# gisbi-kim/navtech-radar-slam

Measured on AMD Instinct MI355X. Metric: sc_loop_queries_per_sec_vs_10k_scan_db, higher is better.
Workload: dtype f16 filter + f64 exact

## Files before the change

### navtech-radar-slam_amd/csrc/sc_window.hip

```cpp
#include <hip/hip_runtime.h>

#include <cmath>
#include <cstdint>

#include "rsx_common.h"
#include "sc_kernels.h"
#include "sc_entry_dev.h"
#include "sc_window_dev.h"

namespace rsx {
namespace sc {

namespace {

using win::half8;
using win::floatx16;
using win::u64;
using win::kNonFinite;
using win::W_STEPS;
using win::W_TILE1;
using win::QK_COPY;
using win::QK_LO;
using win::QK_NORM;
using win::W_LDS;

constexpr int W_ST2_OFF = DS * 2, W_QM_OFF = W_ST2_OFF + 2 * 128 * 2;
static_assert(W_ST2_OFF % 16 == 0 && W_QM_OFF % 8 == 0 && W_QM_OFF + 8 <= 5 * WINDOW_P * 4, "staging fits the arrays it aliases");

#ifndef WIN_OCC
#define WIN_OCC 4
#endif
#ifndef WIN_RING
#define WIN_RING 15
#endif
__global__ __launch_bounds__(256) void sc_win_db_keys_kernel(const double *__restrict__ vkey, int64_t first, int64_t count,
                                                             _Float16 *__restrict__ vk16, float *__restrict__ vk_n) {
  const int lane = threadIdx.x & 63, wave = threadIdx.x >> 6;
  const int64_t it = (int64_t)blockIdx.x * 4 + wave;
  if (it >= count) return;
  dev::win_db_keys_entry(vkey, first + it, vk16, vk_n, lane);
}

struct WindowArgs {
  const char *hnR;
  const char *vk16;
  const float *vk_n;
  const u64 *cmask;
  const float *qdesc;
  const double *qnorm;
  const double *qvkey;
  const RescoreEntry *slist;
  const int32_t *sl_cnt;
  WindowPreview *out;
  WindowSurvivor *surv;
  double eps;
  int32_t k;
};

__global__ __launch_bounds__(256, WIN_OCC) void sc_window_kernel(WindowArgs a) {
  extern __shared__ __attribute__((aligned(16))) char smem[];
  __shared__ float s_ub[WINDOW_HEAD];
  __shared__ int s_pos[WINDOW_P];
  __shared__ int s_n2;
  __shared__ float s_tau;
  __shared__ __attribute__((aligned(16))) char s_rec[5 * WINDOW_P * 4];
  float *const s_lb = reinterpret_cast<float *>(s_rec), *const s_pv = s_lb + WINDOW_P, *const s_cand = s_pv + WINDOW_P;
  int *const s_slot = reinterpret_cast<int *>(s_cand + WINDOW_P), *const s_ks = s_slot + WINDOW_P;
  const int lane = threadIdx.x & 63, wave = __builtin_amdgcn_readfirstlane(threadIdx.x >> 6);
  const int qi = blockIdx.x;
  const int sl_cnt = a.sl_cnt[qi];
  WindowSurvivor *list = a.surv + (int64_t)qi * WINDOW_LIST_STRIDE;
  if (sl_cnt <= 0) {
    if (threadIdx.x == 0) {
      WindowListHeader h;
      h.count = 0;
      h.tau_ub = INFINITY;
      h.n_cand = 0;
      h.n_prev = 0;
      *reinterpret_cast<WindowListHeader *>(list) = h;
    }
    return;
  }
  {
    _Float16 *st = reinterpret_cast<_Float16 *>(s_rec);
    _Float16(*st2)[128] = reinterpret_cast<_Float16(*)[128]>(s_rec + W_ST2_OFF);
    u64 *s_qm = reinterpret_cast<u64 *>(s_rec + W_QM_OFF);
    dev::KeySplit ksplit{};
    if (wave == 0) {
      bool nonzero = false, bad = false;
      if (lane < NS) dev::normalise_column(a.qdesc + (int64_t)qi * DS + lane * NR, a.qnorm[(int64_t)qi * NS + lane], &st[lane * NR], nonzero, bad);
      u64 m = __ballot(nonzero && lane < NS);
      if (__ballot(bad && lane < NS)) m |= kNonFinite;
      if (lane == 0) *s_qm = m;
    } else if (wave == 1) {
      ksplit = win::query_keys_stage(lane < NS ? a.qvkey[(int64_t)qi * NS + lane] : 0.0, st2, lane);
    }
    __syncthreads();
    dev::img_query_image(st, *s_qm, reinterpret_cast<uint4 *>(smem), threadIdx.x, 256);
    win::query_keys_copies(st2, smem + FILTER_QIMG_BYTES, threadIdx.x, 256);
    if (wave == 1) win::query_keys_norms(ksplit, smem + FILTER_QIMG_BYTES, lane);
  }
  __syncthreads();
  const int n = lane & 31, hh = lane >> 5;
  const RescoreEntry *sl = a.slist + (int64_t)qi * RESCORE_SHORTLIST_CAP;
  const u64 qm = *reinterpret_cast<const u64 *>(smem + FILTER_QIMG_MASK_OFF);
  const float nq_key = *reinterpret_cast<const float *>(smem + FILTER_QIMG_BYTES + QK_NORM);
  const float uq_key = *reinterpret_cast<const float *>(smem + FILTER_QIMG_BYTES + QK_NORM + 4);
  const char *ap = smem + ((n & 1) ? (FILTER_QIMG_ODD + 40 * n - 8) : (40 * n)) + 16 * hh;
  const char *kp = smem + FILTER_QIMG_BYTES + (n & 7) * QK_COPY + ((n & ~7) + 8 * hh) * 2;

  auto lane_again = [&]() -> int {
    int t = threadIdx.x;
    asm volatile("" : "+v"(t));
    return t & 31;
  };
  auto do_group = [&](auto pos_of, bool have, int pos_any) -> float {
    const int64_t slot = sl[have ? pos_of() : pos_any].slot;

    floatx16 k0 = {0}, k1 = {0};
    {
      const char *bk = a.vk16 + slot * 256 + 16 * hh;
      half8 bh[4], bl[4];
#pragma unroll
      for (int s = 0; s < 4; s++) {
        bh[s] = *reinterpret_cast<const half8 *>(bk + 32 * s);
        bl[s] = *reinterpret_cast<const half8 *>(bk + 128 + 32 * s);
      }
#pragma unroll
      for (int s = 0; s < 4; s++) {
        const half8 ah0 = *reinterpret_cast<const half8 *>(kp + 32 * s);
        const half8 al0 = *reinterpret_cast<const half8 *>(kp + QK_LO + 32 * s);
        const half8 ah1 = *reinterpret_cast<const half8 *>(kp + 64 + 32 * s);
        const half8 al1 = *reinterpret_cast<const half8 *>(kp + QK_LO + 64 + 32 * s);
        k0 = __builtin_amdgcn_mfma_f32_32x32x16_f16(ah0, bh[s], k0, 0, 0, 0);
        k1 = __builtin_amdgcn_mfma_f32_32x32x16_f16(ah1, bh[s], k1, 0, 0, 0);
        k0 = __builtin_amdgcn_mfma_f32_32x32x16_f16(ah0, bl[s], k0, 0, 0, 0);
        k1 = __builtin_amdgcn_mfma_f32_32x32x16_f16(ah1, bl[s], k1, 0, 0, 0);
        k0 = __builtin_amdgcn_mfma_f32_32x32x16_f16(al0, bh[s], k0, 0, 0, 0);
        k1 = __builtin_amdgcn_mfma_f32_32x32x16_f16(al1, bh[s], k1, 0, 0, 0);
      }
    }
    u64 win;
    int kstar;
    win::alignment_of(k0, k1, nq_key, uq_key, reinterpret_cast<const float2 *>(a.vk_n)[slot], hh, win, kstar);

    __builtin_amdgcn_sched_barrier(0);
    floatx16 acc0 = {0}, acc1 = {0};
    {
      const char *brow = a.hnR + slot * (2 * DS) + 16 * hh;
      constexpr int R = WIN_RING;
      static_assert(W_STEPS % R == 0, "whole ring turns");
      half8 ring[R];
#pragma unroll
      for (int u = 0; u < R; u++) ring[u] = *reinterpret_cast<const half8 *>(brow + 32 * u);
#pragma unroll 1
      for (int s0 = 0; s0 < W_STEPS - R; s0 += R) {
#pragma unroll
        for (int u = 0; u < R; u++) {
          const half8 a0 = *reinterpret_cast<const half8 *>(ap + 32 * (s0 + u));
          const half8 a1 = *reinterpret_cast<const half8 *>(ap + 32 * (s0 + u + W_TILE1));
          acc0 = __builtin_amdgcn_mfma_f32_32x32x16_f16(a0, ring[u], acc0, 0, 0, 0);
          acc1 = __builtin_amdgcn_mfma_f32_32x32x16_f16(a1, ring[u], acc1, 0, 0, 0);
          ring[u] = *reinterpret_cast<const half8 *>(brow + 32 * (s0 + R + u));
        }
      }
#pragma unroll
      for (int u = 0; u < R; u++) {
        const half8 a0 = *reinterpret_cast<const half8 *>(ap + 32 * (W_STEPS - R + u));
        const half8 a1 = *reinterpret_cast<const half8 *>(ap + 32 * (W_STEPS - R + u + W_TILE1));
        acc0 = __builtin_amdgcn_mfma_f32_32x32x16_f16(a0, ring[u], acc0, 0, 0, 0);
        acc1 = __builtin_amdgcn_mfma_f32_32x32x16_f16(a1, ring[u], acc1, 0, 0, 0);
      }
    }

    __builtin_amdgcn_sched_barrier(0);
    const u64 em = a.cmask[slot];
    u64 qmg = qm;
    asm volatile("" : "+v"(qmg));
    const float pv = win::preview_of(acc0, acc1, qmg, em, win, kstar, hh);
    if (have && hh == 0) {
      const int pos = pos_of();
      WindowPreview o;
      o.pv = pv;
      o.ks = kstar;
      a.out[(int64_t)qi * WINDOW_P + pos] = o;
      s_slot[pos] = (int)slot;
      s_pv[pos] = pv;
      s_ks[pos] = kstar;
    }
    return (have && kstar >= 0 && pv < 3.0e38f) ? pv + WINDOW_MARGIN : INFINITY;
  };

  auto write_list = [&](float tau_head, int n2) {
    const int lim = sl_cnt < WINDOW_P ? sl_cnt : WINDOW_P;
    const int nh = lim < WINDOW_HEAD ? lim : WINDOW_HEAD;
    const unsigned long long below = (1ull << lane) - 1ull;
    auto records = [&](auto f) {
      for (int p0 = 0; p0 < nh; p0 += 64) f(p0 + lane, p0 + lane < nh);
      for (int c0 = 0; c0 < n2; c0 += 64) f(c0 + lane < n2 ? s_pos[c0 + lane] : 0, c0 + lane < n2);
    };
    int nc = 0;
    records([&](int pos, bool in) {
      const float pv = s_pv[pos];
      const float ub = pv + WINDOW_MARGIN;
      const bool c = in && s_ks[pos] >= 0 && pv < 3.0e38f && ub <= tau_head;
      const unsigned long long bal = __ballot(c);
      if (c) s_cand[nc + __popcll(bal & below)] = ub;
      nc += __popcll(bal);
    });
    dev::wave_lds_fence();
    float tau_w = INFINITY;
    if (nc >= a.k) {
      for (int c0 = 0; c0 < nc; c0 += 64) {
        const int i = c0 + lane;
        const float v = i < nc ? s_cand[i] : INFINITY;
        int r = 0;
        for (int j = 0; j < nc; j++) {
          const float x = s_cand[j];
          r += (x < v || (x == v && j < i)) ? 1 : 0;
        }
        const unsigned long long b = __ballot(i < nc && r == a.k - 1);
        if (b) {
          tau_w = __shfl(v, __ffsll((long long)b) - 1);
          break;
        }
      }
    }
    int ns = 0, n_cand = 0, n_prev = 0;
    records([&](int pos, bool in) {
      const float pv = s_pv[pos];
      const int ks = s_ks[pos];
      const bool none = in && !(pv == pv);
      const bool lb_ok = !((double)s_lb[pos] - a.eps > (double)tau_w);
      const bool cand = in && (none || (pv < INFINITY && lb_ok));
      const float lo = none ? -INFINITY : pv - WINDOW_MARGIN;
      const bool sv = cand && !(lo > tau_w);
      const unsigned long long bal = __ballot(sv);
      if (sv) {
        WindowSurvivor e;
        e.lo = lo;
        e.slot = s_slot[pos];
        e.ks = (none || ks < 0) ? -1 : ks;
        e.pos = pos;
        list[1 + ns + __popcll(bal & below)] = e;
      }
      ns += __popcll(bal);
      n_cand += __popcll(__ballot(cand));
      n_prev += __popcll(__ballot(cand && !none));
    });
    if (lane == 0) {
      WindowListHeader h;
      h.count = ns;
      h.tau_ub = tau_w;
      h.n_cand = n_cand;
      h.n_prev = n_prev;
      *reinterpret_cast<WindowListHeader *>(list) = h;
    }
  };

  float tau_ub;
  {
    const int cnt1 = sl_cnt < WINDOW_HEAD ? sl_cnt : WINDOW_HEAD;
    float ub = INFINITY;
    if (wave * 32 < cnt1) ub = do_group([&] { return wave * 32 + lane_again(); }, wave * 32 + n < cnt1, wave * 32);
    if (hh == 0) s_ub[wave * 32 + n] = ub;
    __syncthreads();
    float lbh0 = INFINITY, lbh1 = INFINITY;
    if (wave == 0) {
      if (lane < cnt1) lbh0 = sl[lane].lb;
      if (lane + 64 < cnt1) lbh1 = sl[lane + 64].lb;
    }
    if (sl_cnt <= WINDOW_HEAD) {
      if (wave == 0) {
        s_lb[lane] = lbh0;
        s_lb[lane + 64] = lbh1;
        dev::wave_lds_fence();
        write_list(INFINITY, 0);
      }
      return;
    }

    {
      const float v0 = s_ub[lane], v1 = s_ub[lane + 64];
      int r0 = 0, r1 = 0;
      const float4 *u4 = reinterpret_cast<const float4 *>(s_ub);
#pragma unroll 4
      for (int j = 0; j < WINDOW_HEAD / 4; j++) {
        const float4 u = u4[j];
        const float x[4] = {u.x, u.y, u.z, u.w};
#pragma unroll
        for (int e = 0; e < 4; e++) {
          const int idx = 4 * j + e;
          r0 += (x[e] < v0 || (x[e] == v0 && idx < lane)) ? 1 : 0;
          r1 += (x[e] < v1 || (x[e] == v1 && idx < lane + 64)) ? 1 : 0;
        }
      }
      const int want = a.k - 1;
      const unsigned long long b0 = __ballot(r0 == want), b1 = __ballot(r1 == want);
      const float c0 = __shfl(v0, b0 ? __ffsll((long long)b0) - 1 : 0), c1 = __shfl(v1, b1 ? __ffsll((long long)b1) - 1 : 0);
      tau_ub = b0 ? c0 : c1;
    }
    if (wave == 0) {
      s_lb[lane] = lbh0;
      s_lb[lane + 64] = lbh1;
    }
  }
  if (wave == 0) {
    int n2 = 0;
    const int lim = sl_cnt < WINDOW_P ? sl_cnt : WINDOW_P;
    for (int p0 = WINDOW_HEAD; p0 < lim; p0 += 64) {
      const int pos = p0 + lane;
      bool pass = false;
      if (pos < lim) {
        const float lb = sl[pos].lb;
        s_lb[pos] = lb;
        pass = !((double)lb - a.eps > (double)tau_ub);
        if (!pass) {
          WindowPreview o;
          o.pv = __builtin_nanf("");
          o.ks = -2;
          a.out[(int64_t)qi * WINDOW_P + pos] = o;
        }
      }
      const unsigned long long bal = __ballot(pass);
      if (pass) s_pos[n2 + __popcll(bal & ((1ull << lane) - 1ull))] = pos;
      n2 += __popcll(bal);
    }
    if (lane == 0) {
      s_n2 = n2;
      s_tau = tau_ub;
    }
  }
  __syncthreads();
  const int n2 = s_n2;
  for (int g = wave; g * 32 < n2; g += 4) {
    const bool have = g * 32 + n < n2;
    (void)do_group([&] { return s_pos[g * 32 + lane_again()]; }, have, s_pos[g * 32]);
  }
  __syncthreads();
  if (wave == 0) write_list(s_tau, n2);
}

}

int launch_window_db_keys(const double *vkey, int64_t first, int64_t count, void *vk16, float *vk_n, hipStream_t s) {
  if (count <= 0) return RSX_OK;
  hipLaunchKernelGGL(sc_win_db_keys_kernel, dim3((unsigned)((count + 3) / 4)), dim3(256), 0, s, vkey, first, count,
                     static_cast<_Float16 *>(vk16), vk_n);
  RSX_HIP(hipGetLastError());
  return RSX_OK;
}

int launch_window(const DbView &db, const QueryView &q, const RescoreEntry *slist, const int32_t *sl_cnt,
                  int32_t k, double eps, WindowPreview *out, WindowSurvivor *surv, hipStream_t s) {
  if (q.nq <= 0) return RSX_OK;
  WindowArgs a;
  a.hnR = static_cast<const char *>(db.hnR);
  a.vk16 = static_cast<const char *>(db.vk16);
  a.vk_n = db.vk_n;
  a.cmask = reinterpret_cast<const u64 *>(db.cmask);
  a.qdesc = q.desc;
  a.qnorm = q.norm;
  a.qvkey = q.vkey;
  a.slist = slist;
  a.sl_cnt = sl_cnt;
  a.out = out;
  a.surv = surv;
  a.eps = eps;
  a.k = k < 1 ? 1 : (k > WINDOW_HEAD ? WINDOW_HEAD : k);
  hipLaunchKernelGGL(sc_window_kernel, dim3((unsigned)q.nq), dim3(256), W_LDS, s, a);
  RSX_HIP(hipGetLastError());
  return RSX_OK;
}

const char *window_kernel_name() { return "sc_window_kernel"; }

}
}
```

### navtech-radar-slam_amd/csrc/sc_window_dev.h

```cpp
#pragma once
#include <hip/hip_runtime.h>

#include <cmath>
#include <cstdint>

#include "sc_kernels.h"
#include "sc_entry_dev.h"

namespace rsx {
namespace sc {
namespace win {

typedef _Float16 half8 __attribute__((ext_vector_type(8)));
typedef float floatx16 __attribute__((ext_vector_type(16)));
typedef unsigned long long u64;

constexpr float kWinAlignEps = 3e-5f;
constexpr u64 kNonFinite = 1ull << 63;
constexpr int W_STEPS = DS / 16;
constexpr int W_TILE1 = 40;
constexpr int QK_COPY = 288;
constexpr int QK_LO = 8 * QK_COPY;
constexpr int QK_NORM = 2 * QK_LO;
static_assert(QK_NORM + 16 == WINDOW_QK_BYTES, "layout");
constexpr int W_LDS = FILTER_QIMG_BYTES + WINDOW_QK_BYTES;

template <bool DPP = false>
__device__ __forceinline__ dev::KeySplit query_keys_stage(double v, _Float16 (*st)[128], int lane) {
  const dev::KeySplit k = dev::split_key<DPP>(lane < NS ? v : 0.0, lane);
  if (lane < NS) {
    st[0][lane] = k.hi;
    st[1][lane] = k.lo;
    st[0][lane + NS] = k.hi;
    st[1][lane + NS] = k.lo;
  }
  if (lane < 8) {
    st[0][2 * NS + lane] = (_Float16)0.0f;
    st[1][2 * NS + lane] = (_Float16)0.0f;
  }
  return k;
}
__device__ __forceinline__ void query_keys_copies(const _Float16 (*st)[128], char *out, int first, int step) {
  for (int i = first; i < 2 * 8 * (QK_COPY / 2); i += step) {
    const int part = i / (8 * (QK_COPY / 2));
    const int r = i % (8 * (QK_COPY / 2));
    const int c = r / (QK_COPY / 2), el = r % (QK_COPY / 2);
    const int src = c + el;
    const _Float16 v16 = src < 2 * NS ? st[part][src] : (_Float16)0.0f;
    *reinterpret_cast<_Float16 *>(out + part * QK_LO + c * QK_COPY + el * 2) = v16;
  }
}
__device__ __forceinline__ void query_keys_norms(const dev::KeySplit &k, char *out, int lane) {
  if (lane < 4) *reinterpret_cast<float *>(out + QK_NORM + lane * 4) = lane == 0 ? k.nrm : (lane == 1 ? k.unrm : 0.0f);
}

template <bool LEAN = false>
__device__ __forceinline__ void alignment_of(const floatx16 &k0, const floatx16 &k1, float nq_key, float uq_key, float2 en,
                                             int hh, u64 &win, int &kstar) {
  float mx = -INFINITY;
  bool bad = false;
#pragma unroll
  for (int r = 0; r < 16; r++) {
    bad |= !(k0[r] == k0[r]);
    mx = fmaxf(mx, k0[r]);
  }
#pragma unroll
  for (int r = 0; r < 16; r++) {
    const float v = (r >= 12 && hh) ? 0.0f : k1[r];
    bad |= !(v == v);
    mx = fmaxf(mx, (r >= 12 && hh) ? -INFINITY : v);
  }
  float gmx;
  if constexpr (LEAN) {
    const auto sw = __builtin_amdgcn_permlane32_swap(__float_as_uint(mx), __float_as_uint(mx), false, false);
    gmx = fmaxf(__uint_as_float(sw[0]), __uint_as_float(sw[1]));
  } else {
    gmx = fmaxf(mx, __shfl_xor(mx, 32));
  }
  const float thr = 2.0f * kWinAlignEps * nq_key * en.x;
  const float umin = fminf(uq_key, en.y), umax = fmaxf(uq_key, en.y);
  const bool balanced = umin >= 1e-6f * umax && umax < INFINITY && umin > 0.0f;
  const float line = gmx - thr;
  unsigned m0 = 0, m1 = 0;
#pragma unroll
  for (int r = 0; r < 16; r++) m0 |= (k0[r] >= line) ? (1u << ((r & 3) + 8 * (r >> 2))) : 0u;
#pragma unroll
  for (int r = 0; r < 16; r++) m1 |= (k1[r] >= line) ? (1u << ((r & 3) + 8 * (r >> 2))) : 0u;
  m0 <<= 4 * hh;
  m1 <<= 4 * hh;
  bool obad;
  if constexpr (LEAN) {
    const auto s0 = __builtin_amdgcn_permlane32_swap(m0, m0, false, false);
    const auto s1 = __builtin_amdgcn_permlane32_swap(m1, m1, false, false);
    const auto sb = __builtin_amdgcn_permlane32_swap((unsigned)bad, (unsigned)bad, false, false);
    m0 = s0[0] | s0[1];
    m1 = s1[0] | s1[1];
    obad = (sb[0] | sb[1]) != 0;
  } else {
    m0 |= (unsigned)__shfl_xor((int)m0, 32);
    m1 |= (unsigned)__shfl_xor((int)m1, 32);
    obad = __shfl_xor((int)bad, 32) != 0;
  }
  constexpr u64 M60 = (1ull << NS) - 1ull;
  u64 adm = (((u64)m1 << 32) | m0) & M60;
  const bool comparable = !bad && !obad && (thr == thr) && thr < 3.0e38f && balanced && adm != 0;
  if (!comparable) adm = M60;
  kstar = (__popcll(adm) == 1) ? (__ffsll((long long)adm) - 1) : -1;
  win = adm;
#pragma unroll
  for (int o = 1; o <= 3; o++) {
    win |= ((adm << o) | (adm >> (NS - o))) & M60;
    win |= ((adm >> o) | (adm << (NS - o))) & M60;
  }
}

template <bool LEAN = false>
__device__ __forceinline__ float preview_of(floatx16 &acc0, floatx16 &acc1, u64 qm, u64 em, u64 win, int &kstar, int hh) {
  float pv;
  if constexpr (LEAN) {
    constexpr u64 M60 = (1ull << NS) - 1ull;
    const u64 winh = win >> (4 * hh);
    const unsigned wlo = (unsigned)winh, whi = (unsigned)(winh >> 32);
    float best = -INFINITY;
    if ((qm & M60) == M60) {
      const float rn = __builtin_amdgcn_rcpf((float)__popcll(em & M60));
#pragma unroll
      for (int r = 0; r < 16; r++) {
        const int b = (r & 3) + 8 * (r >> 2);
        const float v0 = (wlo & (1u << b)) ? acc0[r] * rn : -INFINITY, v1 = (whi & (1u << b)) ? acc1[r] * rn : -INFINITY;
        acc0[r] = v0;
        acc1[r] = v1;
        best = fmaxf(best, fmaxf(v0, v1));
      }
    } else {
      const u64 m1c = qm & ~kNonFinite;
      const u64 lo = m1c | (m1c << 60), hi = m1c >> 4;
      const u64 lo4 = (lo >> 4) | (hi << 60), hi4 = hi >> 4;
      const u64 l = hh ? lo4 : lo, h = hh ? hi4 : hi;
      const unsigned w[4] = {(unsigned)l, (unsigned)(l >> 32), (unsigned)h, (unsigned)(h >> 32)};
      const unsigned m2lo = (unsigned)em, m2hi = (unsigned)(em >> 32) & 0x0fffffffu;
      auto piece = [&](int tl, int r, float S) -> float {
        const int b = (r & 3) + 8 * (r >> 2);
        const unsigned rlo = __builtin_amdgcn_alignbit(w[tl + 1], w[tl], b);
        const unsigned rhi = __builtin_amdgcn_alignbit(w[tl + 2], w[tl + 1], b);
        const int ne = __builtin_popcount(rlo & m2lo) + __builtin_popcount(rhi & m2hi);
        float v = S * __builtin_amdgcn_rcpf((float)ne);
        v = (((tl ? whi : wlo) >> b) & 1u) ? v : -INFINITY;
        best = fmaxf(best, v);
        return v;
      };
#pragma unroll
      for (int r = 0; r < 16; r++) acc0[r] = piece(0, r, acc0[r]);
#pragma unroll
      for (int r = 0; r < 16; r++) acc1[r] = piece(1, r, acc1[r]);
    }
    {
      const auto sw = __builtin_amdgcn_permlane32_swap(__float_as_uint(best), __float_as_uint(best), false, false);
      best = fmaxf(__uint_as_float(sw[0]), __uint_as_float(sw[1]));
    }
    pv = fmaf(best, -1.0f / FILTER_ACC_SCALE, 1.0f);
    if (kstar >= 0) {
      const float line = best - 2.0f * WINDOW_MARGIN * FILTER_ACC_SCALE;
      unsigned g0 = 0, g1 = 0;
#pragma unroll
      for (int r = 0; r < 16; r++) {
        const int b = (r & 3) + 8 * (r >> 2);
        g0 |= (acc0[r] >= line) ? (1u << b) : 0u;
        g1 |= (acc1[r] >= line) ? (1u << b) : 0u;
      }
      u64 ge = (((u64)g1 << 32) | g0) << (4 * hh);
      {
        const auto sl = __builtin_amdgcn_permlane32_swap((unsigned)ge, (unsigned)ge, false, false);
        const auto sh = __builtin_amdgcn_permlane32_swap((unsigned)(ge >> 32), (unsigned)(ge >> 32), false, false);
        ge = ((u64)(sh[0] | sh[1]) << 32) | (sl[0] | sl[1]);
      }
      int k0s = kstar - 3;
      k0s += k0s < 0 ? NS : 0;
      const unsigned mask7 = (unsigned)((ge >> k0s) | (ge << (NS - k0s))) & 0x7fu;
      kstar |= (int)(mask7 << 8);
    }
  } else {
    const u64 m1c = qm & ~kNonFinite;
    const u64 lo = m1c | (m1c << 60), hi = m1c >> 4;
    const u64 lo4 = (lo >> 4) | (hi << 60), hi4 = hi >> 4;
    const u64 l = hh ? lo4 : lo, h = hh ? hi4 : hi;
    const unsigned w[4] = {(unsigned)l, (unsigned)(l >> 32), (unsigned)h, (unsigned)(h >> 32)};
    const unsigned m2lo = (unsigned)em, m2hi = (unsigned)(em >> 32) & 0x0fffffffu;
    const u64 winh = win >> (4 * hh);
    const unsigned wlo = (unsigned)winh, whi = (unsigned)(winh >> 32);
    float best = -INFINITY;
    auto piece = [&](int tl, int r, float S) -> float {
      const int b = (r & 3) + 8 * (r >> 2);
      const unsigned rlo = __builtin_amdgcn_alignbit(w[tl + 1], w[tl], b);
      const unsigned rhi = __builtin_amdgcn_alignbit(w[tl + 2], w[tl + 1], b);
      const int ne = __builtin_popcount(rlo & m2lo) + __builtin_popcount(rhi & m2hi);
      float v = S * __builtin_amdgcn_rcpf((float)ne);
      const bool inwin = ((tl ? whi : wlo) >> b) & 1u;
      v = inwin ? v : -INFINITY;
      best = fmaxf(best, v);
      return v;
    };
#pragma unroll
    for (int r = 0; r < 16; r++) acc0[r] = piece(0, r, acc0[r]);
#pragma unroll
    for (int r = 0; r < 16; r++) acc1[r] = piece(1, r, acc1[r]);
    best = fmaxf(best, __shfl_xor(best, 32));
    pv = fmaf(best, -1.0f / FILTER_ACC_SCALE, 1.0f);
    if (kstar >= 0) {
      const float line = best - 2.0f * WINDOW_MARGIN * FILTER_ACC_SCALE;
      int k0s = kstar - 3;
      k0s += k0s < 0 ? NS : 0;
      unsigned mask7 = 0;
      auto near = [&](int tl, int r, float v) {
        int t = 32 * tl + (r & 3) + 8 * (r >> 2) + 4 * hh - k0s;
        t += t < 0 ? NS : 0;
        mask7 |= (v >= line && t < 7) ? (1u << t) : 0u;
      };
#pragma unroll
      for (int r = 0; r < 16; r++) near(0, r, acc0[r]);
#pragma unroll
      for (int r = 0; r < 16; r++) near(1, r, acc1[r]);
      mask7 |= (unsigned)__shfl_xor((int)mask7, 32);
      kstar |= (int)(mask7 << 8);
    }
  }
  if ((qm | em) & kNonFinite) pv = __builtin_nanf("");
  return pv;
}

}
}
}
```

Baseline: 3.236 million.

## Prefetch query and shortlist data early, stage slots in LDS, parallelize ranking

Loads the query descriptor columns, norms, keys and shortlist records into registers at kernel entry so their global latency overlaps the early-exit check and staging. Slots and lower bounds are staged into LDS once, replacing repeated global shortlist reads inside groups and selection. The cmask and key-norm loads are hoisted ahead of the MFMA work, and the tau ranking is spread over all four waves with a shuffle reduction instead of one wave doing it. The query-key copy loop gets a fixed 256-thread mapping, and lean variants of the alignment and preview helpers are used. An optional compile-time profiling path is added but is off by default.

```diff
diff --git a/navtech-radar-slam_amd/csrc/sc_window.hip b/navtech-radar-slam_amd/csrc/sc_window.hip
--- a/navtech-radar-slam_amd/csrc/sc_window.hip
+++ b/navtech-radar-slam_amd/csrc/sc_window.hip
@@ -2,6 +2,7 @@
 
 #include <cmath>
 #include <cstdint>
+#include <cstdio>
 
 #include "rsx_common.h"
 #include "sc_kernels.h"
@@ -33,6 +34,25 @@
 #ifndef WIN_RING
 #define WIN_RING 15
 #endif
+#ifdef RSX_WINDOW_PROF
+constexpr bool kWinProf = true;
+#else
+constexpr bool kWinProf = false;
+#endif
+enum WinProfRegion {
+  WP_PROLOGUE = 0,
+  WP_GROUP1,
+  WP_RANK,
+  WP_SELECT,
+  WP_GROUP2,
+  WP_TAIL,
+  WP_BARRIER,
+  WP_TOTAL,
+  WP_COUNT,
+  WP_GROUPS2,
+  WIN_PROF_WORDS
+};
+constexpr int WIN_PROF_COPIES = 64;
 __global__ __launch_bounds__(256) void sc_win_db_keys_kernel(const double *__restrict__ vkey, int64_t first, int64_t count,
                                                              _Float16 *__restrict__ vk16, float *__restrict__ vk_n) {
   const int lane = threadIdx.x & 63, wave = threadIdx.x >> 6;
@@ -55,6 +75,7 @@
   WindowSurvivor *surv;
   double eps;
   int32_t k;
+  unsigned long long *prof;
 };
 
 __global__ __launch_bounds__(256, WIN_OCC) void sc_window_kernel(WindowArgs a) {
@@ -68,6 +89,53 @@
   int *const s_slot = reinterpret_cast<int *>(s_cand + WINDOW_P), *const s_ks = s_slot + WINDOW_P;
   const int lane = threadIdx.x & 63, wave = __builtin_amdgcn_readfirstlane(threadIdx.x >> 6);
   const int qi = blockIdx.x;
+  long long t_mark = 0, t_begin = 0, tacc[WP_TOTAL] = {0, 0, 0, 0, 0, 0, 0};
+  int prof_groups2 = 0;
+  if constexpr (kWinProf) t_begin = t_mark = clock64();
+  auto lap = [&](int region) {
+    if constexpr (kWinProf) {
+      asm volatile("s_waitcnt vmcnt(0) lgkmcnt(0)" ::: "memory");
+      const long long t = clock64();
+      tacc[region] += t - t_mark;
+      t_mark = t;
+    }
+  };
+  auto barrier = [&](int region) {
+    lap(region);
+    __syncthreads();
+    lap(WP_BARRIER);
+  };
+  auto prof_flush = [&]() {
+    if constexpr (kWinProf) {
+      if (a.prof && lane == 0) {
+        unsigned long long *o = a.prof + ((size_t)(qi % WIN_PROF_COPIES) * 4 + wave) * WIN_PROF_WORDS;
+#pragma unroll
+        for (int r = 0; r < WP_TOTAL; r++) atomicAdd(o + r, (unsigned long long)tacc[r]);
+        atomicAdd(o + WP_TOTAL, (unsigned long long)(t_mark - t_begin));
+        atomicAdd(o + WP_COUNT, 1ull);
+        atomicAdd(o + WP_GROUPS2, (unsigned long long)prof_groups2);
+      }
+    }
+  };
+  float4 qcol[5] = {};
+  double qn = 0.0, qv = 0.0;
+  if (wave == 0) {
+    if (lane < NS) {
+      const float4 *p = reinterpret_cast<const float4 *>(a.qdesc + (int64_t)qi * DS + lane * NR);
+#pragma unroll
+      for (int i = 0; i < 5; i++) qcol[i] = p[i];
+      qn = a.qnorm[(int64_t)qi * NS + lane];
+    }
+  } else if (wave == 1) {
+    if (lane < NS) qv = a.qvkey[(int64_t)qi * NS + lane];
+  }
+  static_assert(WINDOW_P <= 2 * 256 && WINDOW_P <= RESCORE_SHORTLIST_CAP, "two positions per thread, inside the query's records");
+  uint2 rec0, rec1 = {0u, 0u};
+  {
+    const uint2 *sl2 = reinterpret_cast<const uint2 *>(a.slist + (int64_t)qi * RESCORE_SHORTLIST_CAP);
+    rec0 = sl2[threadIdx.x];
+    if (threadIdx.x + 256 < WINDOW_P) rec1 = sl2[threadIdx.x + 256];
+  }
   const int sl_cnt = a.sl_cnt[qi];
   WindowSurvivor *list = a.surv + (int64_t)qi * WINDOW_LIST_STRIDE;
   if (sl_cnt <= 0) {
@@ -81,6 +149,8 @@
     }
     return;
   }
+  static_assert(3 * WINDOW_P * 4 >= W_QM_OFF + 8, "s_slot clear of the staging area");
+  const int lim = sl_cnt < WINDOW_P ? sl_cnt : WINDOW_P;
   {
     _Float16 *st = reinterpret_cast<_Float16 *>(s_rec);
     _Float16(*st2)[128] = reinterpret_cast<_Float16(*)[128]>(s_rec + W_ST2_OFF);
@@ -88,21 +158,24 @@
     dev::KeySplit ksplit{};
     if (wave == 0) {
       bool nonzero = false, bad = false;
-      if (lane < NS) dev::normalise_column(a.qdesc + (int64_t)qi * DS + lane * NR, a.qnorm[(int64_t)qi * NS + lane], &st[lane * NR], nonzero, bad);
+      if (lane < NS) dev::normalise_column_regs(qcol, qn, &st[lane * NR], nonzero, bad);
       u64 m = __ballot(nonzero && lane < NS);
       if (__ballot(bad && lane < NS)) m |= kNonFinite;
       if (lane == 0) *s_qm = m;
     } else if (wave == 1) {
-      ksplit = win::query_keys_stage(lane < NS ? a.qvkey[(int64_t)qi * NS + lane] : 0.0, st2, lane);
-    }
-    __syncthreads();
+      ksplit = win::query_keys_stage(lane < NS ? qv : 0.0, st2, lane);
+    }
+    barrier(WP_PROLOGUE);
     dev::img_query_image(st, *s_qm, reinterpret_cast<uint4 *>(smem), threadIdx.x, 256);
-    win::query_keys_copies(st2, smem + FILTER_QIMG_BYTES, threadIdx.x, 256);
+    win::query_keys_copies_256(st2, smem + FILTER_QIMG_BYTES, threadIdx.x);
     if (wave == 1) win::query_keys_norms(ksplit, smem + FILTER_QIMG_BYTES, lane);
   }
-  __syncthreads();
+  if ((int)threadIdx.x < lim) s_slot[threadIdx.x] = (int)rec0.y;
+  if ((int)threadIdx.x + 256 < lim) s_slot[threadIdx.x + 256] = (int)rec1.y;
+  barrier(WP_PROLOGUE);
+  if ((int)threadIdx.x < lim) s_lb[threadIdx.x] = __uint_as_float(rec0.x);
+  if ((int)threadIdx.x + 256 < lim) s_lb[threadIdx.x + 256] = __uint_as_float(rec1.x);
   const int n = lane & 31, hh = lane >> 5;
-  const RescoreEntry *sl = a.slist + (int64_t)qi * RESCORE_SHORTLIST_CAP;
   const u64 qm = *reinterpret_cast<const u64 *>(smem + FILTER_QIMG_MASK_OFF);
   const float nq_key = *reinterpret_cast<const float *>(smem + FILTER_QIMG_BYTES + QK_NORM);
   const float uq_key = *reinterpret_cast<const float *>(smem + FILTER_QIMG_BYTES + QK_NORM + 4);
@@ -115,7 +188,9 @@
     return t & 31;
   };
   auto do_group = [&](auto pos_of, bool have, int pos_any) -> float {
-    const int64_t slot = sl[have ? pos_of() : pos_any].slot;
+    const int64_t slot = s_slot[have ? pos_of() : pos_any];
+    const u64 em = a.cmask[slot];
+    const float2 en = reinterpret_cast<const float2 *>(a.vk_n)[slot];
 
     floatx16 k0 = {0}, k1 = {0};
     {
@@ -142,7 +217,7 @@
     }
     u64 win;
     int kstar;
-    win::alignment_of(k0, k1, nq_key, uq_key, reinterpret_cast<const float2 *>(a.vk_n)[slot], hh, win, kstar);
+    win::alignment_of<true>(k0, k1, nq_key, uq_key, en, hh, win, kstar);
 
     __builtin_amdgcn_sched_barrier(0);
     floatx16 acc0 = {0}, acc1 = {0};
@@ -174,17 +249,15 @@
     }
 
     __builtin_amdgcn_sched_barrier(0);
-    const u64 em = a.cmask[slot];
     u64 qmg = qm;
     asm volatile("" : "+v"(qmg));
-    const float pv = win::preview_of(acc0, acc1, qmg, em, win, kstar, hh);
+    const float pv = win::preview_of<true>(acc0, acc1, qmg, em, win, kstar, hh);
     if (have && hh == 0) {
       const int pos = pos_of();
       WindowPreview o;
       o.pv = pv;
       o.ks = kstar;
       a.out[(int64_t)qi * WINDOW_P + pos] = o;
-      s_slot[pos] = (int)slot;
       s_pv[pos] = pv;
       s_ks[pos] = kstar;
     }
@@ -192,7 +265,6 @@
   };
 
   auto write_list = [&](float tau_head, int n2) {
-    const int lim = sl_cnt < WINDOW_P ? sl_cnt : WINDOW_P;
     const int nh = lim < WINDOW_HEAD ? lim : WINDOW_HEAD;
     const unsigned long long below = (1ull << lane) - 1ull;
     auto records = [&](auto f) {
@@ -264,56 +336,42 @@
     float ub = INFINITY;
     if (wave * 32 < cnt1) ub = do_group([&] { return wave * 32 + lane_again(); }, wave * 32 + n < cnt1, wave * 32);
     if (hh == 0) s_ub[wave * 32 + n] = ub;
-    __syncthreads();
-    float lbh0 = INFINITY, lbh1 = INFINITY;
-    if (wave == 0) {
-      if (lane < cnt1) lbh0 = sl[lane].lb;
-      if (lane + 64 < cnt1) lbh1 = sl[lane + 64].lb;
-    }
+    barrier(WP_GROUP1);
     if (sl_cnt <= WINDOW_HEAD) {
-      if (wave == 0) {
-        s_lb[lane] = lbh0;
-        s_lb[lane + 64] = lbh1;
-        dev::wave_lds_fence();
-        write_list(INFINITY, 0);
-      }
+      if (wave == 0) write_list(INFINITY, 0);
+      lap(WP_TAIL);
+      prof_flush();
       return;
     }
 
     {
-      const float v0 = s_ub[lane], v1 = s_ub[lane + 64];
-      int r0 = 0, r1 = 0;
-      const float4 *u4 = reinterpret_cast<const float4 *>(s_ub);
+      const int p = wave * 32 + n;
+      const float v = s_ub[p];
+      int r = 0;
+      const float4 *u4 = reinterpret_cast<const float4 *>(s_ub) + (WINDOW_HEAD / 8) * hh;
 #pragma unroll 4
-      for (int j = 0; j < WINDOW_HEAD / 4; j++) {
+      for (int j = 0; j < WINDOW_HEAD / 8; j++) {
         const float4 u = u4[j];
         const float x[4] = {u.x, u.y, u.z, u.w};
 #pragma unroll
         for (int e = 0; e < 4; e++) {
-          const int idx = 4 * j + e;
-          r0 += (x[e] < v0 || (x[e] == v0 && idx < lane)) ? 1 : 0;
-          r1 += (x[e] < v1 || (x[e] == v1 && idx < lane + 64)) ? 1 : 0;
+          const int idx = (WINDOW_HEAD / 2) * hh + 4 * j + e;
+          r += (x[e] < v || (x[e] == v && idx < p)) ? 1 : 0;
         }
       }
-      const int want = a.k - 1;
-      const unsigned long long b0 = __ballot(r0 == want), b1 = __ballot(r1 == want);
-      const float c0 = __shfl(v0, b0 ? __ffsll((long long)b0) - 1 : 0), c1 = __shfl(v1, b1 ? __ffsll((long long)b1) - 1 : 0);
-      tau_ub = b0 ? c0 : c1;
-    }
-    if (wave == 0) {
-      s_lb[lane] = lbh0;
-      s_lb[lane + 64] = lbh1;
-    }
+      r += __shfl_xor(r, 32);
+      if (hh == 0 && r == a.k - 1) s_tau = v;
+    }
+    barrier(WP_RANK);
+    tau_ub = s_tau;
   }
   if (wave == 0) {
     int n2 = 0;
-    const int lim = sl_cnt < WINDOW_P ? sl_cnt : WINDOW_P;
     for (int p0 = WINDOW_HEAD; p0 < lim; p0 += 64) {
       const int pos = p0 + lane;
       bool pass = false;
       if (pos < lim) {
-        const float lb = sl[pos].lb;
-        s_lb[pos] = lb;
+        const float lb = s_lb[pos];
         pass = !((double)lb - a.eps > (double)tau_ub);
         if (!pass) {
           WindowPreview o;
@@ -326,19 +384,19 @@
       if (pass) s_pos[n2 + __popcll(bal & ((1ull << lane) - 1ull))] = pos;
       n2 += __popcll(bal);
     }
-    if (lane == 0) {
-      s_n2 = n2;
-      s_tau = tau_ub;
-    }
-  }
-  __syncthreads();
+    if (lane == 0) s_n2 = n2;
+  }
+  barrier(WP_SELECT);
   const int n2 = s_n2;
   for (int g = wave; g * 32 < n2; g += 4) {
     const bool have = g * 32 + n < n2;
     (void)do_group([&] { return s_pos[g * 32 + lane_again()]; }, have, s_pos[g * 32]);
-  }
-  __syncthreads();
+    prof_groups2++;
+  }
+  barrier(WP_GROUP2);
   if (wave == 0) write_list(s_tau, n2);
+  lap(WP_TAIL);
+  prof_flush();
 }
 
 }
@@ -368,8 +426,33 @@
   a.surv = surv;
   a.eps = eps;
   a.k = k < 1 ? 1 : (k > WINDOW_HEAD ? WINDOW_HEAD : k);
+  a.prof = nullptr;
+#ifdef RSX_WINDOW_PROF
+  constexpr size_t kProfWords = (size_t)WIN_PROF_COPIES * 4 * WIN_PROF_WORDS;
+  static unsigned long long *d_prof = nullptr;
+  if (!d_prof) RSX_HIP(hipMalloc(reinterpret_cast<void **>(&d_prof), kProfWords * 8));
+  RSX_HIP(hipMemsetAsync(d_prof, 0, kProfWords * 8, s));
+  a.prof = d_prof;
+#endif
   hipLaunchKernelGGL(sc_window_kernel, dim3((unsigned)q.nq), dim3(256), W_LDS, s, a);
   RSX_HIP(hipGetLastError());
+#ifdef RSX_WINDOW_PROF
+  {
+    static unsigned long long h[kProfWords];
+    RSX_HIP(hipMemcpyAsync(h, d_prof, kProfWords * 8, hipMemcpyDeviceToHost, s));
+    RSX_HIP(hipStreamSynchronize(s));
+    static const char *const names[WP_TOTAL + 1] = {"prologue", "pass-1 group", "ranking", "pass-2 selection", "pass-2 groups", "tail", "barriers", "total"};
+    for (int w = 0; w < 4; w++) {
+      double v[WIN_PROF_WORDS] = {0};
+      for (int c = 0; c < WIN_PROF_COPIES; c++)
+        for (int i = 0; i < WIN_PROF_WORDS; i++) v[i] += (double)h[((size_t)c * 4 + w) * WIN_PROF_WORDS + i];
+      if (v[WP_COUNT] <= 0) continue;
+      fprintf(stderr, "[sc_window prof] nq %d wave %d (cycles per workgroup, %.0f reported, %.3f pass-2 groups):", (int)q.nq, w, v[WP_COUNT], v[WP_GROUPS2] / v[WP_COUNT]);
+      for (int r = 0; r <= WP_TOTAL; r++) fprintf(stderr, "  %s %.0f", names[r], v[r] / v[WP_COUNT]);
+      fprintf(stderr, "\n");
+    }
+  }
+#endif
   return RSX_OK;
 }
 
diff --git a/navtech-radar-slam_amd/csrc/sc_window_dev.h b/navtech-radar-slam_amd/csrc/sc_window_dev.h
--- a/navtech-radar-slam_amd/csrc/sc_window_dev.h
+++ b/navtech-radar-slam_amd/csrc/sc_window_dev.h
@@ -48,6 +48,16 @@
     const int src = c + el;
     const _Float16 v16 = src < 2 * NS ? st[part][src] : (_Float16)0.0f;
     *reinterpret_cast<_Float16 *>(out + part * QK_LO + c * QK_COPY + el * 2) = v16;
+  }
+}
+__device__ __forceinline__ void query_keys_copies_256(const _Float16 (*st)[128], char *out, int tid) {
+  static_assert(QK_COPY / 2 == 16 * 9, "nine elements per thread");
+  const int part = tid >> 7, c = (tid >> 4) & 7;
+  _Float16 *o = reinterpret_cast<_Float16 *>(out + part * QK_LO + c * QK_COPY);
+#pragma unroll
+  for (int j = 0; j < 9; j++) {
+    const int el = (tid & 15) + 16 * j, src = c + el;
+    o[el] = src < 2 * NS ? st[part][src] : (_Float16)0.0f;
   }
 }
 __device__ __forceinline__ void query_keys_norms(const dev::KeySplit &k, char *out, int lane) {
```

Result: faster. 3.277 million, median of 6 (+1.3%).
